# luizirber/sourmash-rust

Hardware: NVIDIA B200
Metric: Gbp/s sketched (higher is better)
Workload: dtype u64

## Files before the change

sourmash_rust_b200/csrc/kmer_bits.cuh:

```cuda
#pragma once
#include <stdint.h>

#if defined(__CUDACC__)
#define KB_HD __host__ __device__ __forceinline__
#else
#define KB_HD inline
#endif

namespace smb200 {

KB_HD uint32_t kb_byte_perm(uint32_t a, uint32_t b, uint32_t sel) {
#if defined(__CUDA_ARCH__)
    return __byte_perm(a, b, sel);
#else
    const uint64_t pool = ((uint64_t)b << 32) | a;
    uint32_t r = 0;
    for (int i = 0; i < 4; i++) {
        const uint32_t s = (sel >> (4 * i)) & 0x7u;
        r |= (uint32_t)((pool >> (8 * s)) & 0xFFu) << (8 * i);
    }
    return r;
#endif
}
KB_HD uint32_t kb_brev(uint32_t x) {
#if defined(__CUDA_ARCH__)
    return __brev(x);
#else
    x = ((x >> 1) & 0x55555555u) | ((x & 0x55555555u) << 1);
    x = ((x >> 2) & 0x33333333u) | ((x & 0x33333333u) << 2);
    x = ((x >> 4) & 0x0F0F0F0Fu) | ((x & 0x0F0F0F0Fu) << 4);
    x = ((x >> 8) & 0x00FF00FFu) | ((x & 0x00FF00FFu) << 8);
    return (x >> 16) | (x << 16);
#endif
}
KB_HD uint32_t kb_funnel_r(uint32_t lo, uint32_t hi, uint32_t s) {
#if defined(__CUDA_ARCH__)
    return __funnelshift_r(lo, hi, s);
#else
    s &= 31u;
    return s ? ((lo >> s) | (hi << (32 - s))) : lo;
#endif
}

struct Quad {
    uint32_t upper;
    uint32_t comp;
    uint32_t codes8;
    uint32_t bad4;
};
KB_HD Quad classify4(uint32_t raw) {
    Quad q;
    const uint32_t u = raw & 0xDFDFDFDFu;
    const uint32_t c = ((u >> 1) ^ (u >> 2)) & 0x03030303u;
    const uint32_t sel = (c & 0x3u) | ((c >> 4) & 0x30u) | ((c >> 8) & 0x300u) | ((c >> 12) & 0x3000u);
    const uint32_t expect = kb_byte_perm(0x54474341u , 0u, sel);
    const uint32_t x = expect ^ u;
    const uint32_t nz = (x | ((x & 0x7F7F7F7Fu) + 0x7F7F7F7Fu)) & 0x80808080u;
    q.upper = u;
    q.comp = kb_byte_perm(0x41434754u , 0u, sel);
    q.codes8 = (c * 0x01041040u) >> 24;
    q.bad4 = ((nz >> 7) * 0x01020408u) >> 24;
    return q;
}

KB_HD uint32_t pair_reverse16(uint32_t x) {
    x = kb_brev(x) >> 16;
    return ((x >> 1) & 0x5555u) | ((x & 0x5555u) << 1);
}

struct Oct {
    uint32_t fA0, fA1;
    uint32_t rA0, rA1;
    uint32_t f2;
    uint32_t r2;
    uint32_t bad8;
};
KB_HD Oct classify8(uint32_t raw0, uint32_t raw1) {
    const Quad a = classify4(raw0), b = classify4(raw1);
    Oct o;
    o.fA0 = a.upper;
    o.fA1 = b.upper;
    o.rA0 = kb_byte_perm(b.comp, 0u, 0x0123u);
    o.rA1 = kb_byte_perm(a.comp, 0u, 0x0123u);
    o.f2 = a.codes8 | (b.codes8 << 8);
    o.r2 = (~pair_reverse16(o.f2)) & 0xFFFFu;
    o.bad8 = a.bad4 | (b.bad4 << 4);
    return o;
}

template <int K>
struct KmerGeom {
    static constexpr int NE = (2 * K + 31) / 32;
    static constexpr int NW = (K + 3) / 4;
    static constexpr uint32_t TOP2 = (2 * K) % 32 ? ((1u << ((2 * K) % 32)) - 1u) : 0xFFFFFFFFu;
    static constexpr uint32_t TOPA = (K % 4) ? ((1u << ((K % 4) * 8)) - 1u) : 0xFFFFFFFFu;
};

template <int K>
KB_HD void extract2(const uint32_t *stream, int start, uint32_t (&e)[KmerGeom<K>::NE]) {
    const int w = start >> 4;
    const uint32_t s = (uint32_t)(start & 15) * 2u;
    uint32_t prev = stream[w];
#pragma unroll
    for (int j = 0; j < KmerGeom<K>::NE; j++) {
        const uint32_t next = stream[w + j + 1];
        e[j] = kb_funnel_r(prev, next, s);
        prev = next;
    }
    e[KmerGeom<K>::NE - 1] &= KmerGeom<K>::TOP2;
}

template <int K>
KB_HD void extract2w(const uint32_t *w, uint32_t s, uint32_t (&e)[KmerGeom<K>::NE]) {
    uint32_t prev = w[0];
#pragma unroll
    for (int j = 0; j < KmerGeom<K>::NE; j++) {
        const uint32_t next = w[j + 1];
        e[j] = kb_funnel_r(prev, next, s);
        prev = next;
    }
    e[KmerGeom<K>::NE - 1] &= KmerGeom<K>::TOP2;
}

template <int K>
KB_HD void extract2_end(const uint32_t *w, uint32_t s, uint32_t (&e)[KmerGeom<K>::NE]) {
    static_assert(K % 2 == 1, "end-aligned strand comparison needs an odd k");
    uint32_t prev = w[0];
#pragma unroll
    for (int j = 0; j < KmerGeom<K>::NE; j++) {
        const uint32_t next = w[j + 1];
        e[j] = kb_funnel_r(prev, next, s);
        prev = next;
    }
}

template <int K>
KB_HD bool canonical_is_fw(const uint32_t (&ef)[KmerGeom<K>::NE], const uint32_t (&er)[KmerGeom<K>::NE]) {
    constexpr int NE = KmerGeom<K>::NE;
    if (NE == 1) return ef[0] < er[0];
    if (NE == 2) return (((uint64_t)ef[1] << 32) | ef[0]) < (((uint64_t)er[1] << 32) | er[0]);
    bool lt = false;
#pragma unroll
    for (int j = 0; j < NE; j++) {
        if (ef[j] != er[j]) lt = ef[j] < er[j];
    }
    return lt;
}

template <int K>
KB_HD void extractA(const uint32_t *words, int start, uint32_t (&kw)[KmerGeom<K>::NW]) {
    const int w = start >> 2;
    const uint32_t s = (uint32_t)(start & 3) * 8u;
    uint32_t prev = words[w];
#pragma unroll
    for (int j = 0; j < KmerGeom<K>::NW; j++) {
        const uint32_t next = words[w + j + 1];
        kw[j] = kb_funnel_r(prev, next, s);
        prev = next;
    }
    kw[KmerGeom<K>::NW - 1] &= KmerGeom<K>::TOPA;
}

template <int K>
KB_HD void extractAw(const uint32_t *w, uint32_t s, uint32_t (&kw)[KmerGeom<K>::NW]) {
    uint32_t prev = w[0];
#pragma unroll
    for (int j = 0; j < KmerGeom<K>::NW; j++) {
        const uint32_t next = w[j + 1];
        kw[j] = kb_funnel_r(prev, next, s);
        prev = next;
    }
    kw[KmerGeom<K>::NW - 1] &= KmerGeom<K>::TOPA;
}

KB_HD void kb_shr96(uint32_t &x0, uint32_t &x1, uint32_t &x2, int s) {
    if (s < 32) {
        x0 = kb_funnel_r(x0, x1, (uint32_t)s);
        x1 = kb_funnel_r(x1, x2, (uint32_t)s);
        x2 >>= s;
    } else {
        x0 = kb_funnel_r(x1, x2, (uint32_t)(s - 32));
        x1 = (s == 32) ? x2 : (x2 >> (s - 32));
        x2 = 0;
    }
}
KB_HD uint32_t dilate_word(uint32_t in0, uint32_t in1, uint32_t in2, int span) {
    if (span <= 0) return 0;
    uint32_t d0 = in0, d1 = in1, d2 = in2;
    int a = 1;
    while (2 * a <= span) {
        uint32_t y0 = d0, y1 = d1, y2 = d2;
        kb_shr96(y0, y1, y2, a);
        d0 |= y0; d1 |= y1; d2 |= y2;
        a *= 2;
    }
    if (span > a) {
        uint32_t y0 = d0, y1 = d1, y2 = d2;
        kb_shr96(y0, y1, y2, span - a);
        d0 |= y0;
    }
    return d0;
}

}
```

sourmash_rust_b200/csrc/murmur3.cuh:

```cuda
#pragma once
#include <stdint.h>

#if defined(__CUDACC__)
#define SM_HD __host__ __device__ __forceinline__
#else
#define SM_HD inline
#endif

namespace smb200 {

constexpr uint64_t MM_C1 = 0x87c37b91114253d5ULL;
constexpr uint64_t MM_C2 = 0x4cf5ad432745937fULL;

template <uint64_t C>
SM_HD uint64_t mm_mulc(uint64_t x) {
#if defined(__CUDA_ARCH__)
    uint64_t r;
    asm("{\n\t.reg .u32 lo, hi, rl, rh;\n\t.reg .u64 t;\n\t"
        "mov.b64 {lo, hi}, %1;\n\t"
        "mul.wide.u32 t, lo, %2;\n\t"
        "mov.b64 {rl, rh}, t;\n\t"
        "mad.lo.u32 rh, lo, %3, rh;\n\t"
        "mad.lo.u32 rh, hi, %2, rh;\n\t"
        "mov.b64 %0, {rl, rh};\n\t}"
        : "=l"(r)
        : "l"(x), "n"((uint32_t)C), "n"((uint32_t)(C >> 32)));
    return r;
#else
    return x * C;
#endif
}
template <uint32_t ADD>
SM_HD uint64_t mm_mul5add(uint64_t x) {
#if defined(__CUDA_ARCH__) && defined(MM_MUL5_WIDE)
    uint64_t r;
    asm("{\n\t.reg .u32 lo, hi, rl, rh;\n\t.reg .u64 t;\n\t"
        "mov.b64 {lo, hi}, %1;\n\t"
        "mad.wide.u32 t, lo, 5, %2;\n\t"
        "mov.b64 {rl, rh}, t;\n\t"
        "mad.lo.u32 rh, hi, 5, rh;\n\t"
        "mov.b64 %0, {rl, rh};\n\t}"
        : "=l"(r)
        : "l"(x), "l"((uint64_t)ADD));
    return r;
#else
    return x * 5 + ADD;
#endif
}
template <int R>
SM_HD uint64_t mm_rotl64(uint64_t x) {
#if defined(__CUDA_ARCH__)
    const uint32_t lo = (uint32_t)x, hi = (uint32_t)(x >> 32);
    constexpr uint32_t S = (uint32_t)(R & 31);
    uint32_t nlo, nhi;
    if (R < 32) { nhi = __funnelshift_l(lo, hi, S); nlo = __funnelshift_l(hi, lo, S); }
    else        { nhi = __funnelshift_l(hi, lo, S); nlo = __funnelshift_l(lo, hi, S); }
    return ((uint64_t)nhi << 32) | nlo;
#else
    return (x << R) | (x >> (64 - R));
#endif
}

SM_HD uint64_t mm_xorshift33(uint64_t k) {
#if defined(__CUDA_ARCH__) && defined(MM_XS_IMADHI)
    uint32_t lo = (uint32_t)k, hi = (uint32_t)(k >> 32), t;
    asm("mul.hi.u32 %0, %1, 0x80000000;" : "=r"(t) : "r"(hi));
    lo ^= t;
    return ((uint64_t)hi << 32) | lo;
#else
    return k ^ (k >> 33);
#endif
}
SM_HD uint64_t mm_fmix64(uint64_t k) {
    k = mm_xorshift33(k);
    k = mm_mulc<0xff51afd7ed558ccdULL>(k);
    k = mm_xorshift33(k);
    k = mm_mulc<0xc4ceb9fe1a85ec53ULL>(k);
    k = mm_xorshift33(k);
    return k;
}

SM_HD uint64_t mm_mix_k1(uint64_t k1) {
    k1 = mm_mulc<MM_C1>(k1); k1 = mm_rotl64<31>(k1); k1 = mm_mulc<MM_C2>(k1);
    return k1;
}
SM_HD uint64_t mm_mix_k2(uint64_t k2) {
    k2 = mm_mulc<MM_C2>(k2); k2 = mm_rotl64<33>(k2); k2 = mm_mulc<MM_C1>(k2);
    return k2;
}
SM_HD void mm_body(uint64_t &h1, uint64_t &h2, uint64_t k1, uint64_t k2) {
    h1 ^= mm_mix_k1(k1);
    h1 = mm_rotl64<27>(h1); h1 += h2; h1 = mm_mul5add<0x52dce729u>(h1);
    h2 ^= mm_mix_k2(k2);
    h2 = mm_rotl64<31>(h2); h2 += h1; h2 = mm_mul5add<0x38495ab5u>(h2);
}
SM_HD uint64_t mm_final_h1(uint64_t h1, uint64_t h2, uint64_t len) {
    h1 ^= len; h2 ^= len;
    h1 += h2; h2 += h1;
    h1 = mm_fmix64(h1); h2 = mm_fmix64(h2);
    h1 += h2;
    return h1;
}

SM_HD uint64_t murmur3_h1_bytes(const uint8_t *data, uint64_t len, uint64_t seed) {
    uint64_t h1 = seed, h2 = seed;
    const uint64_t nblocks = len / 16;
    for (uint64_t b = 0; b < nblocks; b++) {
        uint64_t k1 = 0, k2 = 0;
        for (int j = 7; j >= 0; j--) {
            k1 = (k1 << 8) | data[16 * b + j];
            k2 = (k2 << 8) | data[16 * b + 8 + j];
        }
        mm_body(h1, h2, k1, k2);
    }
    const uint8_t *tail = data + nblocks * 16;
    const int rem = (int)(len & 15);
    uint64_t k1 = 0, k2 = 0;
    for (int j = rem - 1; j >= 8; j--) k2 = (k2 << 8) | tail[j];
    for (int j = (rem < 8 ? rem : 8) - 1; j >= 0; j--) k1 = (k1 << 8) | tail[j];
    if (rem > 8) h2 ^= mm_mix_k2(k2);
    if (rem > 0) h1 ^= mm_mix_k1(k1);
    return mm_final_h1(h1, h2, len);
}

template <int K>
SM_HD uint64_t murmur3_h1_words(const uint32_t *w, uint64_t seed) {
    constexpr int NB = K / 16;
    constexpr int REM = K % 16;
    uint64_t h1 = seed, h2 = seed;
#pragma unroll
    for (int b = 0; b < NB; b++) {
        const uint64_t k1 = ((uint64_t)w[4 * b + 1] << 32) | w[4 * b + 0];
        const uint64_t k2 = ((uint64_t)w[4 * b + 3] << 32) | w[4 * b + 2];
        mm_body(h1, h2, k1, k2);
    }
    if (REM > 8) {
        const uint32_t hi = (REM > 12) ? w[4 * NB + 3] : 0u;
        const uint64_t k2 = ((uint64_t)hi << 32) | w[4 * NB + 2];
        h2 ^= mm_mix_k2(k2);
    }
    if (REM > 0) {
        const uint32_t hi = (REM > 4) ? w[4 * NB + 1] : 0u;
        const uint64_t k1 = ((uint64_t)hi << 32) | w[4 * NB + 0];
        h1 ^= mm_mix_k1(k1);
    }
    return mm_final_h1(h1, h2, (uint64_t)K);
}

}
```

sourmash_rust_b200/csrc/sketch.cu:

```cuda
#include "device.hpp"
#include "kernels.cuh"
#include "kmer_bits.cuh"
#include "murmur3.cuh"

namespace smb200 {

#ifndef SK_UNROLL
#define SK_UNROLL 4
#endif
#ifndef SK_SHIFTED
#define SK_SHIFTED 1
#endif
#ifndef SK_UNROLL_FUSED
#define SK_UNROLL_FUSED 2
#endif
#ifndef SK_MIN_CTAS
#define SK_MIN_CTAS SK_CTAS_PER_SM
#endif

__device__ __forceinline__ uint32_t smem_u32(const void *p) { return (uint32_t)__cvta_generic_to_shared(p); }
__device__ __forceinline__ void mbar_init(uint64_t *bar, uint32_t count) {
    asm volatile("mbarrier.init.shared::cta.b64 [%0], %1;" ::"r"(smem_u32(bar)), "r"(count));
    asm volatile("fence.mbarrier_init.release.cluster;" ::: "memory");
}
__device__ __forceinline__ void mbar_expect_tx(uint64_t *bar, uint32_t bytes) {
    asm volatile("mbarrier.arrive.expect_tx.shared::cta.b64 _, [%0], %1;" ::"r"(smem_u32(bar)), "r"(bytes)
                 : "memory");
}
__device__ __forceinline__ void mbar_wait(uint64_t *bar, uint32_t parity) {
    asm volatile(
        "{\n\t"
        ".reg .pred p;\n\t"
        "WAIT_%=:\n\t"
        "mbarrier.try_wait.parity.shared::cta.b64 p, [%0], %1;\n\t"
        "@p bra DONE_%=;\n\t"
        "bra WAIT_%=;\n\t"
        "DONE_%=:\n\t"
        "}" ::"r"(smem_u32(bar)),
        "r"(parity)
        : "memory");
}
__device__ __forceinline__ void tma_load_1d(void *dst, const void *src, uint32_t bytes, uint64_t *bar) {
    asm volatile(
        "cp.async.bulk.shared::cluster.global.mbarrier::complete_tx::bytes [%0], [%1], %2, [%3];" ::"r"(
            smem_u32(dst)),
        "l"(src), "r"(bytes), "r"(smem_u32(bar))
        : "memory");
}

struct TileViews {
    uint8_t *raw;
    uint32_t *fA;
    uint32_t *rA;
    uint32_t *f2;
    uint32_t *r2;
    uint32_t *bad;
    uint32_t *end;
    uint32_t *sbad;
};
constexpr int SK_PAD2 = 4;
__host__ __device__ constexpr int tile_bases(int K) { return SK_TILE + ((K - 1 + 15) / 16) * 16; }
__host__ __device__ constexpr int copy_stride_words(int B) {
    int w = (B + 8) / 4 + 4;
    while (w % 32 != 8) w++;
    return w;
}
__host__ __device__ constexpr size_t tile_smem_bytes(int B, int nk = 1) {
    return (size_t)B
           + (SK_SHIFTED ? 8 * (size_t)copy_stride_words(B) * 4 : 2 * ((size_t)B + 16))
           + 2 * ((size_t)B / 4 + 8 + 4 * SK_PAD2)
           + 2 * ((size_t)(B + 31) / 32 * 4 + 12)
           + (size_t)nk * (SK_TILE / 8)
           + 128;
}
__device__ __forceinline__ TileViews carve_tile(uint8_t *base, int B) {
    TileViews v;
    uint8_t *p = base;
    v.raw = p; p += B;
    v.fA = reinterpret_cast<uint32_t *>(p); p += SK_SHIFTED ? 16 * copy_stride_words(B) : (B + 16);
    v.rA = reinterpret_cast<uint32_t *>(p); p += SK_SHIFTED ? 16 * copy_stride_words(B) : (B + 16);
    v.f2 = reinterpret_cast<uint32_t *>(p) + SK_PAD2; p += B / 4 + 8 + 4 * SK_PAD2;
    v.r2 = reinterpret_cast<uint32_t *>(p) + SK_PAD2; p += B / 4 + 8 + 4 * SK_PAD2;
    const int wm = (B + 31) / 32 + 3;
    v.bad = reinterpret_cast<uint32_t *>(p); p += wm * 4;
    v.end = reinterpret_cast<uint32_t *>(p); p += wm * 4;
    v.sbad = reinterpret_cast<uint32_t *>(p);
    return v;
}

__device__ __forceinline__ uint32_t tile_copy_bytes(uint64_t t0, uint64_t n, int B) {
    if (t0 >= n) return 0;
    const uint64_t left = ((n - t0) + 15) & ~15ull;
    return (uint32_t)(left < (uint64_t)B ? left : (uint64_t)B);
}

__device__ __forceinline__ void build_views(const TileViews &v, int B, uint64_t t0, const SketchBatch &sb) {
    const int tid = threadIdx.x, nthr = blockDim.x;
    const int wm = (B + 31) / 32 + 3;
    for (int w = tid; w < wm; w += nthr) v.end[w] = 0;
    for (int w = (B + 31) / 32 + tid; w < wm; w += nthr) v.bad[w] = 0xFFFFFFFFu;
    if (tid < 2) {
        v.fA[B / 4 + tid] = 0; v.rA[B / 4 + tid] = 0; v.f2[B / 16 + tid] = 0; v.r2[B / 16 + tid] = 0;
    }
    if (tid < SK_PAD2) { v.f2[-1 - tid] = 0; v.r2[-1 - tid] = 0; }
    const uint4 *raw128 = reinterpret_cast<const uint4 *>(v.raw);
    uint4 *fA128 = reinterpret_cast<uint4 *>(v.fA), *rA128 = reinterpret_cast<uint4 *>(v.rA);
    uint16_t *badh = reinterpret_cast<uint16_t *>(v.bad);
    const int groups = B / 16;
    for (int g = tid; g < groups; g += nthr) {
        const uint4 raw = raw128[g];
        const Oct o1 = classify8(raw.x, raw.y), o2 = classify8(raw.z, raw.w);
        uint32_t bad16 = o1.bad8 | (o2.bad8 << 8);
        const uint64_t b0 = t0 + (uint64_t)g * 16;
        if (b0 + 16 > sb.n) bad16 |= (b0 >= sb.n) ? 0xFFFFu : (0xFFFFu << (uint32_t)(sb.n - b0)) & 0xFFFFu;
        fA128[g] = make_uint4(o1.fA0, o1.fA1, o2.fA0, o2.fA1);
        const int rg = groups - 1 - g;
        rA128[rg] = make_uint4(o2.rA0, o2.rA1, o1.rA0, o1.rA1);
        v.f2[g] = o1.f2 | (o2.f2 << 16);
        v.r2[rg] = o2.r2 | (o1.r2 << 16);
        badh[g] = (uint16_t)bad16;
    }
    if (B % 32) {
        if (tid == 0) reinterpret_cast<uint16_t *>(v.bad)[B / 16] = 0xFFFFu;
    }
}

__device__ __forceinline__ void build_shifted_copies(const TileViews &v, int B) {
    const int quads = (B / 4 + 1 + 3) / 4, stride4 = copy_stride_words(B) / 4;
    for (int q = threadIdx.x; q < 2 * quads; q += blockDim.x) {
        uint32_t *x = (q < quads) ? v.fA : v.rA;
        const int j = (q < quads) ? q : q - quads;
        const uint4 a = reinterpret_cast<const uint4 *>(x)[j];
        const uint32_t n = x[4 * j + 4];
        uint4 *c = reinterpret_cast<uint4 *>(x);
#pragma unroll
        for (int s = 1; s < 4; s++)
            c[s * stride4 + j] = make_uint4(kb_funnel_r(a.x, a.y, 8 * s), kb_funnel_r(a.y, a.z, 8 * s), kb_funnel_r(a.z, a.w, 8 * s),
                                            kb_funnel_r(a.w, n, 8 * s));
    }
}

__device__ __forceinline__ void mark_sequence_ends(const TileViews &v, int B, uint64_t t0, const SketchBatch &sb) {
    const int tid = threadIdx.x, nthr = blockDim.x;
    const uint64_t hi = t0 + (uint64_t)B;
    if (sb.offsets == nullptr && sb.read_len == 0) {
        if (tid == 0 && sb.n - 1 >= t0 && sb.n - 1 < hi) {
            const uint32_t j = (uint32_t)(sb.n - 1 - t0);
            atomicOr(&v.end[j >> 5], 1u << (j & 31));
        }
    } else if (sb.offsets == nullptr) {
        if (tid < 32) {
            const uint64_t L = sb.read_len;
            uint64_t m = (t0 + 1 + L - 1) / L;
            if (m == 0) m = 1;
            for (m += tid;; m += 32) {
                const uint64_t e = m * L - 1;
                if (e >= hi || e >= sb.n) break;
                const uint32_t j = (uint32_t)(e - t0);
                atomicOr(&v.end[j >> 5], 1u << (j & 31));
            }
        }
    } else {
        uint64_t a = 0, b = sb.n_seqs;
        while (a < b) {
            const uint64_t mid = (a + b) >> 1;
            if (sb.offsets[mid + 1] > t0) b = mid; else a = mid + 1;
        }
        for (uint64_t s = a + tid; s < sb.n_seqs; s += nthr) {
            const uint64_t e1 = sb.offsets[s + 1];
            if (e1 - 1 >= hi) break;
            const uint32_t j = (uint32_t)(e1 - 1 - t0);
            atomicOr(&v.end[j >> 5], 1u << (j & 31));
        }
    }
}

__device__ __forceinline__ void build_start_bitmap(const TileViews &v, uint32_t *sbad, int K, uint64_t t0,
                                                   const SketchBatch &sb, unsigned long long *first_bad) {
    for (int w = threadIdx.x; w < SK_TILE / 32; w += blockDim.x) {
        uint32_t hasbad, crosses;
        if (K <= 64) {
            hasbad = dilate_word(v.bad[w], v.bad[w + 1], v.bad[w + 2], K);
            crosses = dilate_word(v.end[w], v.end[w + 1], v.end[w + 2], K - 1);
        } else {
            hasbad = 0; crosses = 0;
            for (int p = 0; p < 32; p++) {
                const int q = w * 32 + p;
                bool hb = false, cr = false;
                for (int j = q; j < q + K; j++) {
                    const uint32_t bit = 1u << (j & 31);
                    hb |= (v.bad[j >> 5] & bit) != 0;
                    if (j < q + K - 1) cr |= (v.end[j >> 5] & bit) != 0;
                }
                hasbad |= (uint32_t)hb << p;
                crosses |= (uint32_t)cr << p;
            }
        }
        const uint64_t q0 = t0 + (uint64_t)w * 32;
        uint32_t beyond = 0;
        if (q0 + 32 > sb.n_limit) beyond = (q0 >= sb.n_limit) ? 0xFFFFFFFFu : (0xFFFFFFFFu << (uint32_t)(sb.n_limit - q0));
        sbad[w] = hasbad | crosses | beyond;
        const uint32_t err = hasbad & ~crosses & ~beyond;
        if (err && first_bad)
            atomicMin(first_bad, (unsigned long long)(sb.pos_base + q0 + (uint32_t)(__ffs(err) - 1)));
    }
}

__device__ __forceinline__ void append_survivor(bool pass, uint64_t h, uint64_t pos0, const SketchBatch &sb,
                                                const SketchOut &out) {
    if (pass) {
        unsigned lane, tid;
        asm volatile("mov.u32 %0, %%laneid;" : "=r"(lane));
        asm volatile("mov.u32 %0, %%tid.x;" : "=r"(tid));
        const unsigned grp = __activemask();
        const int leader = __ffs(grp) - 1;
        unsigned long long base = 0;
        if ((int)lane == leader) base = atomicAdd(out.counter, (unsigned long long)__popc(grp));
        base = __shfl_sync(grp, base, leader);
        const unsigned long long idx = base + __popc(grp & ((1u << lane) - 1u));
        if (idx < out.cap) {
            out.hash[idx] = h;
            if (out.pos) out.pos[idx] = sb.pos_base + pos0 + tid;
        }
    }
}

template <int K, int B, int UNROLL>
__device__ __forceinline__ void kmer_loop(const TileViews &v, const uint32_t *sbad, const uint64_t thr, const uint64_t t0,
                                          const SketchBatch &sb, const SketchOut &out) {
    using G = KmerGeom<K>;
    static_assert(SK_THREADS % 32 == 0 && 16 * G::NE - K <= 16 * SK_PAD2, "k-mer loop addressing");
    const int tid = threadIdx.x;
    const int ri0 = B - K - tid, ra0 = B + 16 + ri0;
    const int ef0 = tid + K - 16 * G::NE, er0 = ri0 + K - 16 * G::NE;
    const uint32_t *qf2 = v.f2 + (ef0 >> 4), *qr2 = v.r2 + (er0 >> 4);
#if SK_SHIFTED
    constexpr int CS = copy_stride_words(B);
    const uint32_t *qfa = v.fA + (tid & 3) * CS + (tid >> 2), *qra = v.rA + (ri0 & 3) * CS + (ri0 >> 2);
    (void)ra0;
#else
    const uint32_t *qfa = v.fA + (tid >> 2), *qra = v.fA + (ra0 >> 2);
    const uint32_t sfa = (uint32_t)tid * 8u, sra = (uint32_t)ra0 * 8u;
#endif
    const uint32_t sf2 = (uint32_t)ef0 * 2u, sr2 = (uint32_t)er0 * 2u;
    const uint32_t *qsb = sbad + (tid >> 5);
    uint32_t mb = 1u << (tid & 31);
    asm("" : "+r"(mb));
#pragma unroll 1
    for (int r = 0; r < SK_TILE / SK_THREADS; r += UNROLL) {
#pragma unroll
        for (int u = 0; u < UNROLL; u++) {
            const bool valid = (qsb[u * (SK_THREADS / 32)] & mb) == 0;
            uint32_t ef[G::NE], er[G::NE];
            extract2_end<K>(qf2 + u * (SK_THREADS / 16), sf2, ef);
            extract2_end<K>(qr2 - u * (SK_THREADS / 16), sr2, er);
            const bool use_fw = canonical_is_fw<K>(ef, er);
            uint32_t kw[G::NW];
            const uint32_t *pa = use_fw ? qfa + u * (SK_THREADS / 4) : qra - u * (SK_THREADS / 4);
#if SK_SHIFTED
#pragma unroll
            for (int j = 0; j < G::NW; j++) kw[j] = pa[j];
            kw[G::NW - 1] &= G::TOPA;
#else
            extractAw<K>(pa, use_fw ? sfa : sra, kw);
#endif
            const uint64_t h = murmur3_h1_words<K>(kw, sb.seed);
            append_survivor(valid && h <= thr, h, t0 + (uint32_t)((r + u) * SK_THREADS), sb, out);
        }
        qf2 += UNROLL * (SK_THREADS / 16); qr2 -= UNROLL * (SK_THREADS / 16);
        qfa += UNROLL * (SK_THREADS / 4);  qra -= UNROLL * (SK_THREADS / 4);
        qsb += UNROLL * (SK_THREADS / 32);
    }
}

__host__ __device__ constexpr int kmax3(int a, int b, int c) { return a > b ? (a > c ? a : c) : (b > c ? b : c); }

template <int KA, int KB, int KC>
__global__ void __launch_bounds__(SK_THREADS, SK_MIN_CTAS) sketch_kernel(const SketchBatch sb, const SketchOuts outs,
                                                                         uint32_t n_tiles) {
    constexpr int B = tile_bases(kmax3(KA, KB, KC));
    extern __shared__ __align__(128) uint8_t s_dyn[];
    __shared__ __align__(8) uint64_t s_bar;
    const TileViews v = carve_tile(s_dyn, B);
    const int tid = threadIdx.x;
    const uint64_t thrA = *outs.o[0].thr;
    const uint64_t thrB = KB ? *outs.o[1].thr : 0;
    const uint64_t thrC = KC ? *outs.o[2].thr : 0;

    __shared__ uint32_t s_next;
    if (tid == 0) {
        mbar_init(&s_bar, 1);
        s_next = sb.tile_lo + gridDim.x + atomicAdd(sb.tile_ctr, 1u);
    }
    __syncthreads();
    uint32_t tile = sb.tile_lo + blockIdx.x;
    uint32_t parity = 0;
    if (tid == 0 && tile < n_tiles) {
        const uint64_t t0 = (uint64_t)tile * SK_TILE;
        const uint32_t bytes = tile_copy_bytes(t0, sb.n, B);
        mbar_expect_tx(&s_bar, bytes);
        if (bytes) tma_load_1d(v.raw, sb.buf + t0, bytes, &s_bar);
    }
    while (tile < n_tiles) {
        const uint64_t t0 = (uint64_t)tile * SK_TILE;
        const uint32_t next = s_next;
        uint32_t after_next = 0;
        mbar_wait(&s_bar, parity);
        parity ^= 1u;
        build_views(v, B, t0, sb);
        __syncthreads();
        if (tid == 0) {
            if (next < n_tiles) {
                const uint64_t n0 = (uint64_t)next * SK_TILE;
                const uint32_t bytes = tile_copy_bytes(n0, sb.n, B);
                mbar_expect_tx(&s_bar, bytes);
                if (bytes) tma_load_1d(v.raw, sb.buf + n0, bytes, &s_bar);
                after_next = sb.tile_lo + gridDim.x + atomicAdd(sb.tile_ctr, 1u);
            } else {
                after_next = next;
            }
        }
        mark_sequence_ends(v, B, t0, sb);
#if SK_SHIFTED
        build_shifted_copies(v, B);
#endif
        __syncthreads();
        build_start_bitmap(v, v.sbad, KA, t0, sb, outs.first_bad[0]);
        if (KB) build_start_bitmap(v, v.sbad + SK_TILE / 32, KB, t0, sb, outs.first_bad[1]);
        if (KC) build_start_bitmap(v, v.sbad + 2 * (SK_TILE / 32), KC, t0, sb, outs.first_bad[2]);
        __syncthreads();
        constexpr int U = KB ? SK_UNROLL_FUSED : SK_UNROLL;
        kmer_loop<KA, B, U>(v, v.sbad, thrA, t0, sb, outs.o[0]);
        if (KB) kmer_loop<(KB ? KB : KA), B, U>(v, v.sbad + SK_TILE / 32, thrB, t0, sb, outs.o[1]);
        if (KC) kmer_loop<(KC ? KC : KA), B, U>(v, v.sbad + 2 * (SK_TILE / 32), thrC, t0, sb, outs.o[2]);
        if (tid == 0) s_next = after_next;
        __syncthreads();
        tile = next;
    }
    if (tid == 0) {
        __threadfence();
        if (atomicAdd(sb.tile_ctr + 1, 1u) == gridDim.x - 1) {
            sb.tile_ctr[0] = 0;
            sb.tile_ctr[1] = 0;
            __threadfence();
        }
    }
}

__global__ void __launch_bounds__(SK_THREADS) sketch_generic_kernel(const SketchBatch sb, const SketchOut out,
                                                                    uint32_t n_tiles, int K) {
    const int B = SK_TILE + ((K - 1 + 15) / 16) * 16;
    extern __shared__ __align__(128) uint8_t s_dyn[];
    __shared__ __align__(8) uint64_t s_bar;
    const TileViews v = carve_tile(s_dyn, B);
    const int tid = threadIdx.x, lane = tid & 31;
    const uint64_t thr = *out.thr;
    if (tid == 0) mbar_init(&s_bar, 1);
    __syncthreads();
    uint32_t parity = 0;
    for (uint32_t tile = sb.tile_lo + blockIdx.x; tile < n_tiles; tile += gridDim.x) {
        const uint64_t t0 = (uint64_t)tile * SK_TILE;
        if (tid == 0) {
            const uint32_t bytes = tile_copy_bytes(t0, sb.n, B);
            mbar_expect_tx(&s_bar, bytes);
            if (bytes) tma_load_1d(v.raw, sb.buf + t0, bytes, &s_bar);
        }
        mbar_wait(&s_bar, parity);
        parity ^= 1u;
        build_views(v, B, t0, sb);
        __syncthreads();
        mark_sequence_ends(v, B, t0, sb);
        __syncthreads();
        build_start_bitmap(v, v.sbad, K, t0, sb, sb.first_bad);
        __syncthreads();
        const uint8_t *fA = reinterpret_cast<const uint8_t *>(v.fA);
        const uint8_t *rA = reinterpret_cast<const uint8_t *>(v.rA);
        for (int r = 0; r < SK_TILE / SK_THREADS; r++) {
            const int i = r * SK_THREADS + tid;
            const bool valid = ((v.sbad[i >> 5] >> (i & 31)) & 1u) == 0;
            uint64_t h = 0;
            if (valid) {
                const uint8_t *f = fA + i;
                const uint8_t *rc = rA + (B - K - i);
                int j = 0;
                while (j < K && f[j] == rc[j]) j++;
                const uint8_t *src = (j < K && f[j] < rc[j]) ? f : rc;
                h = murmur3_h1_bytes(src, (uint64_t)K, sb.seed);
            }
            append_survivor(valid && h <= thr, h, t0 + (uint32_t)(r * SK_THREADS), sb, out);
        }
        __syncthreads();
    }
}

bool sketch_has_fast_path(uint32_t K) { return K == 21 || K == 31 || K == 51; }
bool sketch_multi_supported(const uint32_t *ks, int nk) {
    if (nk < 2 || nk > 3) return false;
    for (int i = 0; i < nk; i++) {
        if (!sketch_has_fast_path(ks[i])) return false;
        if (i && ks[i] <= ks[i - 1]) return false;
    }
    return true;
}

template <int KA, int KB, int KC>
static void launch_fast(const SketchBatch &sb, const SketchOuts &outs, uint32_t n_tiles, unsigned grid, cudaStream_t st) {
    constexpr int NK = 1 + (KB ? 1 : 0) + (KC ? 1 : 0);
    constexpr size_t smem = tile_smem_bytes(tile_bases(kmax3(KA, KB, KC)), NK);
    static bool attr_set = false;
    if (!attr_set) {
        SM_CUDA(cudaFuncSetAttribute(sketch_kernel<KA, KB, KC>, cudaFuncAttributeMaxDynamicSharedMemorySize, (int)smem));
        attr_set = true;
    }
    sketch_kernel<KA, KB, KC><<<grid, SK_THREADS, smem, st>>>(sb, outs, n_tiles);
}

uint32_t sketch_tile_count(uint64_t n, uint64_t n_limit) {
    const uint64_t span = n_limit < n ? n_limit : n;
    const uint64_t tiles64 = (span + SK_TILE - 1) / SK_TILE;
    if (tiles64 > 0xFFFFFFFFull) throw_internal("sequence batch too large for one launch");
    return (uint32_t)tiles64;
}
uint32_t sketch_tiles_ready(uint32_t K, uint64_t bytes_ready) {
    const uint64_t B = SK_TILE + (((uint64_t)K - 1 + 15) / 16) * 16;
    if (bytes_ready < B) return 0;
    return (uint32_t)((bytes_ready - B) / SK_TILE + 1);
}

static unsigned sketch_grid(const SketchBatch &sb, uint32_t tile_hi, int sm_count) {
    unsigned grid = (unsigned)sm_count * SK_CTAS_PER_SM;
    if (grid > tile_hi - sb.tile_lo) grid = tile_hi - sb.tile_lo;
    return grid;
}

void launch_sketch(uint32_t K, const SketchBatch &sb, const SketchOut &out, uint32_t tile_hi, int sm_count,
                   cudaStream_t st) {
    if (sb.n == 0 || sb.n_limit == 0 || K == 0 || tile_hi <= sb.tile_lo) return;
    const uint32_t n_tiles = tile_hi;
    const unsigned grid = sketch_grid(sb, tile_hi, sm_count);
    ProfScope prof(K == 21 ? PROF_SKETCH_K21 : K == 31 ? PROF_SKETCH_K31 : K == 51 ? PROF_SKETCH_K51 : PROF_SKETCH_OTHER, st);
    SketchOuts outs;
    outs.o[0] = out; outs.o[1] = out; outs.o[2] = out;
    outs.first_bad[0] = sb.first_bad; outs.first_bad[1] = nullptr; outs.first_bad[2] = nullptr;
    switch (K) {
    case 21: launch_fast<21, 0, 0>(sb, outs, n_tiles, grid, st); break;
    case 31: launch_fast<31, 0, 0>(sb, outs, n_tiles, grid, st); break;
    case 51: launch_fast<51, 0, 0>(sb, outs, n_tiles, grid, st); break;
    default: {
        if (K > (uint32_t)SK_MAX_GENERIC_K) throw_internal("ksize above 8192 is not supported by the GPU sketcher");
        const int B = SK_TILE + (((int)K - 1 + 15) / 16) * 16;
        const size_t smem = tile_smem_bytes(B);
        SM_CUDA(cudaFuncSetAttribute(sketch_generic_kernel, cudaFuncAttributeMaxDynamicSharedMemorySize, (int)smem));
        sketch_generic_kernel<<<grid, SK_THREADS, smem, st>>>(sb, out, n_tiles, (int)K);
    }
    }
    SM_LAUNCHED();
}

void launch_sketch_multi(const uint32_t *ks, int nk, const SketchBatch &sb, const SketchOuts &outs, uint32_t tile_hi,
                         int sm_count, cudaStream_t st) {
    if (!sketch_multi_supported(ks, nk)) throw_internal("unsupported k-size combination for the fused sketch kernel");
    if (sb.n == 0 || sb.n_limit == 0 || tile_hi <= sb.tile_lo) return;
    const unsigned grid = sketch_grid(sb, tile_hi, sm_count);
    ProfScope prof(PROF_SKETCH_MULTI, st);
    if (nk == 3) launch_fast<21, 31, 51>(sb, outs, tile_hi, grid, st);
    else if (ks[0] == 21 && ks[1] == 31) launch_fast<21, 31, 0>(sb, outs, tile_hi, grid, st);
    else if (ks[0] == 21 && ks[1] == 51) launch_fast<21, 51, 0>(sb, outs, tile_hi, grid, st);
    else launch_fast<31, 51, 0>(sb, outs, tile_hi, grid, st);
    SM_LAUNCHED();
}

}
```

Before: 54.62.

## Share premixed murmur3 block words across k-sizes in fused 21/31/51 sketch kernel

For the fused k=21,31,51 kernel, each sub-tile now builds a shared-memory table of murmur3 k1/k2 mixes for every 8-byte-aligned forward and reverse-complement window. All three k-size loops then read these premixed words instead of recomputing the multiply-rotate mixes per k-mer, leaving only the tail bytes to mix inline. This drops the shifted-copy buffers for that path, adds per-sub-tile syncs and a larger smem footprint, and clamps the grid by the occupancy query.

```diff
diff --git a/sourmash_rust_b200/csrc/kmer_bits.cuh b/sourmash_rust_b200/csrc/kmer_bits.cuh
--- a/sourmash_rust_b200/csrc/kmer_bits.cuh
+++ b/sourmash_rust_b200/csrc/kmer_bits.cuh
@@ -173,6 +173,17 @@
     kw[KmerGeom<K>::NW - 1] &= KmerGeom<K>::TOPA;
 }
 
+template <int N>
+KB_HD uint64_t kb_bytes64(const uint32_t *w, uint32_t s) {
+    static_assert(N >= 1 && N <= 8, "1 to 8 bytes");
+    constexpr uint32_t LO = N >= 4 ? 0xFFFFFFFFu : (1u << (8 * N)) - 1u;
+    constexpr uint32_t HI = N <= 4 ? 0u : N == 8 ? 0xFFFFFFFFu : (1u << (8 * (N - 4))) - 1u;
+    const uint32_t x0 = w[0], x1 = w[1];
+    const uint32_t lo = kb_funnel_r(x0, x1, s) & LO;
+    const uint32_t hi = HI ? kb_funnel_r(x1, w[2], s) & HI : 0u;
+    return ((uint64_t)hi << 32) | lo;
+}
+
 KB_HD void kb_shr96(uint32_t &x0, uint32_t &x1, uint32_t &x2, int s) {
     if (s < 32) {
         x0 = kb_funnel_r(x0, x1, (uint32_t)s);
diff --git a/sourmash_rust_b200/csrc/murmur3.cuh b/sourmash_rust_b200/csrc/murmur3.cuh
--- a/sourmash_rust_b200/csrc/murmur3.cuh
+++ b/sourmash_rust_b200/csrc/murmur3.cuh
@@ -88,11 +88,14 @@
     k2 = mm_mulc<MM_C2>(k2); k2 = mm_rotl64<33>(k2); k2 = mm_mulc<MM_C1>(k2);
     return k2;
 }
+SM_HD void mm_body_mixed(uint64_t &h1, uint64_t &h2, uint64_t m1, uint64_t m2) {
+    h1 ^= m1;
+    h1 = mm_rotl64<27>(h1); h1 += h2; h1 = mm_mul5add<0x52dce729u>(h1);
+    h2 ^= m2;
+    h2 = mm_rotl64<31>(h2); h2 += h1; h2 = mm_mul5add<0x38495ab5u>(h2);
+}
 SM_HD void mm_body(uint64_t &h1, uint64_t &h2, uint64_t k1, uint64_t k2) {
-    h1 ^= mm_mix_k1(k1);
-    h1 = mm_rotl64<27>(h1); h1 += h2; h1 = mm_mul5add<0x52dce729u>(h1);
-    h2 ^= mm_mix_k2(k2);
-    h2 = mm_rotl64<31>(h2); h2 += h1; h2 = mm_mul5add<0x38495ab5u>(h2);
+    mm_body_mixed(h1, h2, mm_mix_k1(k1), mm_mix_k2(k2));
 }
 SM_HD uint64_t mm_final_h1(uint64_t h1, uint64_t h2, uint64_t len) {
     h1 ^= len; h2 ^= len;
@@ -147,4 +150,33 @@
     return mm_final_h1(h1, h2, (uint64_t)K);
 }
 
+struct MixPair {
+    uint64_t m1, m2;
+};
+SM_HD MixPair mm_mix_pair(uint64_t w0, uint64_t w1) {
+    MixPair e;
+    e.m1 = mm_mix_k1(w0);
+    e.m2 = mm_mix_k2(w1);
+    return e;
 }
+template <int K>
+struct PremixGeom {
+    static constexpr int NB = K / 16;
+    static constexpr int REM = K % 16;
+    static constexpr int NM = 2 * NB + (REM >= 8 ? 1 : 0);
+    static constexpr int TAIL_OFF = 8 * NM;
+    static constexpr int TAIL_LEN = K % 8;
+};
+template <int K>
+SM_HD uint64_t murmur3_h1_premixed(const uint64_t *m, uint64_t tail, uint64_t seed) {
+    using G = PremixGeom<K>;
+    uint64_t h1 = seed, h2 = seed;
+#pragma unroll
+    for (int b = 0; b < G::NB; b++) mm_body_mixed(h1, h2, m[2 * b], m[2 * b + 1]);
+    if (G::REM > 8) h2 ^= mm_mix_k2(tail);
+    if (G::REM >= 8) h1 ^= m[2 * G::NB];
+    else if (G::REM > 0) h1 ^= mm_mix_k1(tail);
+    return mm_final_h1(h1, h2, (uint64_t)K);
+}
+
+}
diff --git a/sourmash_rust_b200/csrc/sketch.cu b/sourmash_rust_b200/csrc/sketch.cu
--- a/sourmash_rust_b200/csrc/sketch.cu
+++ b/sourmash_rust_b200/csrc/sketch.cu
@@ -1,3 +1,5 @@
+#include <mutex>
+
 #include "device.hpp"
 #include "kernels.cuh"
 #include "kmer_bits.cuh"
@@ -16,6 +18,12 @@
 #endif
 #ifndef SK_MIN_CTAS
 #define SK_MIN_CTAS SK_CTAS_PER_SM
+#endif
+#ifndef SK_MIX_W
+#define SK_MIX_W 1024
+#endif
+#ifndef SK_MIX_UNROLL
+#define SK_MIX_UNROLL 4
 #endif
 
 __device__ __forceinline__ uint32_t smem_u32(const void *p) { return (uint32_t)__cvta_generic_to_shared(p); }
@@ -65,20 +73,20 @@
     while (w % 32 != 8) w++;
     return w;
 }
-__host__ __device__ constexpr size_t tile_smem_bytes(int B, int nk = 1) {
+__host__ __device__ constexpr size_t tile_smem_bytes(int B, int nk = 1, bool shifted = SK_SHIFTED) {
     return (size_t)B
-           + (SK_SHIFTED ? 8 * (size_t)copy_stride_words(B) * 4 : 2 * ((size_t)B + 16))
+           + (shifted ? 8 * (size_t)copy_stride_words(B) * 4 : 2 * ((size_t)B + 16))
            + 2 * ((size_t)B / 4 + 8 + 4 * SK_PAD2)
            + 2 * ((size_t)(B + 31) / 32 * 4 + 12)
            + (size_t)nk * (SK_TILE / 8)
            + 128;
 }
-__device__ __forceinline__ TileViews carve_tile(uint8_t *base, int B) {
+__device__ __forceinline__ TileViews carve_tile(uint8_t *base, int B, bool shifted = SK_SHIFTED) {
     TileViews v;
     uint8_t *p = base;
     v.raw = p; p += B;
-    v.fA = reinterpret_cast<uint32_t *>(p); p += SK_SHIFTED ? 16 * copy_stride_words(B) : (B + 16);
-    v.rA = reinterpret_cast<uint32_t *>(p); p += SK_SHIFTED ? 16 * copy_stride_words(B) : (B + 16);
+    v.fA = reinterpret_cast<uint32_t *>(p); p += shifted ? 16 * copy_stride_words(B) : (B + 16);
+    v.rA = reinterpret_cast<uint32_t *>(p); p += shifted ? 16 * copy_stride_words(B) : (B + 16);
     v.f2 = reinterpret_cast<uint32_t *>(p) + SK_PAD2; p += B / 4 + 8 + 4 * SK_PAD2;
     v.r2 = reinterpret_cast<uint32_t *>(p) + SK_PAD2; p += B / 4 + 8 + 4 * SK_PAD2;
     const int wm = (B + 31) / 32 + 3;
@@ -275,13 +283,96 @@
 
 __host__ __device__ constexpr int kmax3(int a, int b, int c) { return a > b ? (a > c ? a : c) : (b > c ? b : c); }
 
+__host__ __device__ constexpr bool sketch_uses_mix_table(int KA, int KB, int KC) { return KA == 21 && KB == 31 && KC == 51; }
+__host__ __device__ constexpr int mix_reach(int K) { return K <= 0 ? -(1 << 20) : (K % 16 >= 8 ? 16 * (K / 16) : 16 * (K / 16 - 1)); }
+__host__ __device__ constexpr int mix_rc_reach(int K) { return K <= 0 ? -(1 << 20) : mix_reach(K) - K; }
+template <int KA, int KB, int KC, int W>
+struct MixTile {
+    static constexpr int KMAX = kmax3(KA, KB, KC);
+    static constexpr int NF = W + kmax3(mix_reach(KA), mix_reach(KB), mix_reach(KC));
+    static constexpr int NR = W + KMAX + kmax3(mix_rc_reach(KA), mix_rc_reach(KB), mix_rc_reach(KC));
+    static constexpr int NT = NF + NR;
+    static constexpr size_t BYTES = ((size_t)NT * sizeof(MixPair) + 127) / 128 * 128;
+    __host__ __device__ static constexpr int rc_entry0(int K) { return NF + W - 1 + KMAX - K; }
+};
+
+template <int B, int NF, int NT>
+__device__ __forceinline__ void build_mix_table(const TileViews &v, MixPair *tab, int a, int rc_lo) {
+    for (int e = threadIdx.x; e < NT; e += blockDim.x) {
+        const int p = e < NF ? a + e : (B + 16) + rc_lo + (e - NF);
+        const uint32_t *w = v.fA + (p >> 2);
+        const uint32_t s = (uint32_t)p * 8u;
+        tab[e] = mm_mix_pair(kb_bytes64<8>(w, s), kb_bytes64<8>(w + 2, s));
+    }
+}
+
+template <int K, int B, int UNROLL, int W, int RC0>
+__device__ __forceinline__ void mix_loop(const TileViews &v, const MixPair *tab, const uint32_t *sbad, const uint64_t thr,
+                                         const uint64_t t0, const int a, const SketchBatch &sb, const SketchOut &out) {
+    using G = KmerGeom<K>;
+    using P = PremixGeom<K>;
+    static_assert(SK_THREADS % 32 == 0 && 16 * G::NE - K <= 16 * SK_PAD2, "k-mer loop addressing");
+    static_assert(W % (SK_THREADS * UNROLL) == 0 && SK_TILE % W == 0, "sub-tile shape");
+    const int tid = threadIdx.x;
+    const int i0 = a + tid, ri0 = B - K - i0, ra0 = B + 16 + ri0;
+    const int ef0 = i0 + K - 16 * G::NE, er0 = ri0 + K - 16 * G::NE;
+    const uint32_t *qf2 = v.f2 + (ef0 >> 4), *qr2 = v.r2 + (er0 >> 4);
+    const uint32_t sf2 = (uint32_t)ef0 * 2u, sr2 = (uint32_t)er0 * 2u;
+    const uint32_t *qfa = v.fA + (i0 >> 2) + P::TAIL_OFF / 4, *qra = v.fA + (ra0 >> 2) + P::TAIL_OFF / 4;
+    const uint32_t sfa = (uint32_t)i0 * 8u, sra = (uint32_t)ra0 * 8u;
+    const MixPair *tf = tab + tid, *tr = tab + RC0 - tid;
+    const uint32_t *qsb = sbad + (i0 >> 5);
+    uint32_t mb = 1u << (tid & 31);
+    asm("" : "+r"(mb));
+#pragma unroll 1
+    for (int r = 0; r < W / SK_THREADS; r += UNROLL) {
+#pragma unroll
+        for (int u = 0; u < UNROLL; u++) {
+            const bool valid = (qsb[u * (SK_THREADS / 32)] & mb) == 0;
+            uint32_t ef[G::NE], er[G::NE];
+            extract2_end<K>(qf2 + u * (SK_THREADS / 16), sf2, ef);
+            extract2_end<K>(qr2 - u * (SK_THREADS / 16), sr2, er);
+            const bool use_fw = canonical_is_fw<K>(ef, er);
+            const MixPair *pt = use_fw ? tf + u * SK_THREADS : tr - u * SK_THREADS;
+            uint64_t m[P::NM];
+#pragma unroll
+            for (int b = 0; b < P::NB; b++) {
+                const MixPair e = pt[16 * b];
+                m[2 * b] = e.m1;
+                m[2 * b + 1] = e.m2;
+            }
+            if (P::NM > 2 * P::NB) m[2 * P::NB] = pt[16 * P::NB].m1;
+            uint64_t tail = 0;
+            if (P::TAIL_LEN)
+                tail = kb_bytes64<(P::TAIL_LEN ? P::TAIL_LEN : 1)>(use_fw ? qfa + u * (SK_THREADS / 4) : qra - u * (SK_THREADS / 4),
+                                                                   use_fw ? sfa : sra);
+            const uint64_t h = murmur3_h1_premixed<K>(m, tail, sb.seed);
+            append_survivor(valid && h <= thr, h, t0 + (uint32_t)(a + (r + u) * SK_THREADS), sb, out);
+        }
+        qf2 += UNROLL * (SK_THREADS / 16); qr2 -= UNROLL * (SK_THREADS / 16);
+        qfa += UNROLL * (SK_THREADS / 4);  qra -= UNROLL * (SK_THREADS / 4);
+        tf += UNROLL * SK_THREADS;         tr -= UNROLL * SK_THREADS;
+        qsb += UNROLL * (SK_THREADS / 32);
+    }
+}
+
+template <int KA, int KB, int KC>
+__host__ __device__ constexpr size_t sketch_smem_bytes() {
+    return sketch_uses_mix_table(KA, KB, KC)
+               ? MixTile<KA, KB, KC, SK_MIX_W>::BYTES + tile_smem_bytes(tile_bases(kmax3(KA, KB, KC)), 1 + (KB ? 1 : 0) + (KC ? 1 : 0), false)
+               : tile_smem_bytes(tile_bases(kmax3(KA, KB, KC)), 1 + (KB ? 1 : 0) + (KC ? 1 : 0));
+}
+
 template <int KA, int KB, int KC>
 __global__ void __launch_bounds__(SK_THREADS, SK_MIN_CTAS) sketch_kernel(const SketchBatch sb, const SketchOuts outs,
                                                                          uint32_t n_tiles) {
     constexpr int B = tile_bases(kmax3(KA, KB, KC));
+    constexpr bool MIX = sketch_uses_mix_table(KA, KB, KC);
+    using MT = MixTile<KA, KB, KC, SK_MIX_W>;
     extern __shared__ __align__(128) uint8_t s_dyn[];
     __shared__ __align__(8) uint64_t s_bar;
-    const TileViews v = carve_tile(s_dyn, B);
+    MixPair *const tab = reinterpret_cast<MixPair *>(s_dyn);
+    const TileViews v = MIX ? carve_tile(s_dyn + MT::BYTES, B, false) : carve_tile(s_dyn, B);
     const int tid = threadIdx.x;
     const uint64_t thrA = *outs.o[0].thr;
     const uint64_t thrB = KB ? *outs.o[1].thr : 0;
@@ -321,20 +412,31 @@
             }
         }
         mark_sequence_ends(v, B, t0, sb);
-#if SK_SHIFTED
-        build_shifted_copies(v, B);
-#endif
+        if (SK_SHIFTED && !MIX) build_shifted_copies(v, B);
         __syncthreads();
         build_start_bitmap(v, v.sbad, KA, t0, sb, outs.first_bad[0]);
         if (KB) build_start_bitmap(v, v.sbad + SK_TILE / 32, KB, t0, sb, outs.first_bad[1]);
         if (KC) build_start_bitmap(v, v.sbad + 2 * (SK_TILE / 32), KC, t0, sb, outs.first_bad[2]);
-        __syncthreads();
-        constexpr int U = KB ? SK_UNROLL_FUSED : SK_UNROLL;
-        kmer_loop<KA, B, U>(v, v.sbad, thrA, t0, sb, outs.o[0]);
-        if (KB) kmer_loop<(KB ? KB : KA), B, U>(v, v.sbad + SK_TILE / 32, thrB, t0, sb, outs.o[1]);
-        if (KC) kmer_loop<(KC ? KC : KA), B, U>(v, v.sbad + 2 * (SK_TILE / 32), thrC, t0, sb, outs.o[2]);
-        if (tid == 0) s_next = after_next;
-        __syncthreads();
+        if constexpr (MIX) {
+            if (tid == 0) s_next = after_next;
+            constexpr int W = SK_MIX_W, KB_ = KB ? KB : KA, KC_ = KC ? KC : KA;
+            for (int a = 0; a < SK_TILE; a += W) {
+                build_mix_table<B, MT::NF, MT::NT>(v, tab, a, B - a - W + 1 - MT::KMAX);
+                __syncthreads();
+                mix_loop<KA, B, SK_MIX_UNROLL, W, MT::rc_entry0(KA)>(v, tab, v.sbad, thrA, t0, a, sb, outs.o[0]);
+                if (KB) mix_loop<KB_, B, SK_MIX_UNROLL, W, MT::rc_entry0(KB_)>(v, tab, v.sbad + SK_TILE / 32, thrB, t0, a, sb, outs.o[1]);
+                if (KC) mix_loop<KC_, B, SK_MIX_UNROLL, W, MT::rc_entry0(KC_)>(v, tab, v.sbad + 2 * (SK_TILE / 32), thrC, t0, a, sb, outs.o[2]);
+                __syncthreads();
+            }
+        } else {
+            __syncthreads();
+            constexpr int U = KB ? SK_UNROLL_FUSED : SK_UNROLL;
+            kmer_loop<KA, B, U>(v, v.sbad, thrA, t0, sb, outs.o[0]);
+            if (KB) kmer_loop<(KB ? KB : KA), B, U>(v, v.sbad + SK_TILE / 32, thrB, t0, sb, outs.o[1]);
+            if (KC) kmer_loop<(KC ? KC : KA), B, U>(v, v.sbad + 2 * (SK_TILE / 32), thrC, t0, sb, outs.o[2]);
+            if (tid == 0) s_next = after_next;
+            __syncthreads();
+        }
         tile = next;
     }
     if (tid == 0) {
@@ -403,16 +505,25 @@
     return true;
 }
 
+static unsigned sketch_grid(const SketchBatch &sb, uint32_t tile_hi, int sm_count, int ctas_per_sm = SK_CTAS_PER_SM) {
+    unsigned grid = (unsigned)sm_count * ctas_per_sm;
+    if (grid > tile_hi - sb.tile_lo) grid = tile_hi - sb.tile_lo;
+    return grid;
+}
+
 template <int KA, int KB, int KC>
-static void launch_fast(const SketchBatch &sb, const SketchOuts &outs, uint32_t n_tiles, unsigned grid, cudaStream_t st) {
-    constexpr int NK = 1 + (KB ? 1 : 0) + (KC ? 1 : 0);
-    constexpr size_t smem = tile_smem_bytes(tile_bases(kmax3(KA, KB, KC)), NK);
-    static bool attr_set = false;
-    if (!attr_set) {
+static void launch_fast(const SketchBatch &sb, const SketchOuts &outs, uint32_t tile_hi, int sm_count, cudaStream_t st) {
+    constexpr size_t smem = sketch_smem_bytes<KA, KB, KC>();
+    static std::once_flag attr_once;
+    static int ctas = SK_CTAS_PER_SM;
+    std::call_once(attr_once, [] {
         SM_CUDA(cudaFuncSetAttribute(sketch_kernel<KA, KB, KC>, cudaFuncAttributeMaxDynamicSharedMemorySize, (int)smem));
-        attr_set = true;
-    }
-    sketch_kernel<KA, KB, KC><<<grid, SK_THREADS, smem, st>>>(sb, outs, n_tiles);
+        int n = 0;
+        SM_CUDA(cudaOccupancyMaxActiveBlocksPerMultiprocessor(&n, sketch_kernel<KA, KB, KC>, SK_THREADS, smem));
+        if (n < 1) throw_internal("sketch kernel does not fit on an SM");
+        if (n < ctas) ctas = n;
+    });
+    sketch_kernel<KA, KB, KC><<<sketch_grid(sb, tile_hi, sm_count, ctas), SK_THREADS, smem, st>>>(sb, outs, tile_hi);
 }
 
 uint32_t sketch_tile_count(uint64_t n, uint64_t n_limit) {
@@ -427,31 +538,24 @@
     return (uint32_t)((bytes_ready - B) / SK_TILE + 1);
 }
 
-static unsigned sketch_grid(const SketchBatch &sb, uint32_t tile_hi, int sm_count) {
-    unsigned grid = (unsigned)sm_count * SK_CTAS_PER_SM;
-    if (grid > tile_hi - sb.tile_lo) grid = tile_hi - sb.tile_lo;
-    return grid;
-}
-
 void launch_sketch(uint32_t K, const SketchBatch &sb, const SketchOut &out, uint32_t tile_hi, int sm_count,
                    cudaStream_t st) {
     if (sb.n == 0 || sb.n_limit == 0 || K == 0 || tile_hi <= sb.tile_lo) return;
     const uint32_t n_tiles = tile_hi;
-    const unsigned grid = sketch_grid(sb, tile_hi, sm_count);
     ProfScope prof(K == 21 ? PROF_SKETCH_K21 : K == 31 ? PROF_SKETCH_K31 : K == 51 ? PROF_SKETCH_K51 : PROF_SKETCH_OTHER, st);
     SketchOuts outs;
     outs.o[0] = out; outs.o[1] = out; outs.o[2] = out;
     outs.first_bad[0] = sb.first_bad; outs.first_bad[1] = nullptr; outs.first_bad[2] = nullptr;
     switch (K) {
-    case 21: launch_fast<21, 0, 0>(sb, outs, n_tiles, grid, st); break;
-    case 31: launch_fast<31, 0, 0>(sb, outs, n_tiles, grid, st); break;
-    case 51: launch_fast<51, 0, 0>(sb, outs, n_tiles, grid, st); break;
+    case 21: launch_fast<21, 0, 0>(sb, outs, n_tiles, sm_count, st); break;
+    case 31: launch_fast<31, 0, 0>(sb, outs, n_tiles, sm_count, st); break;
+    case 51: launch_fast<51, 0, 0>(sb, outs, n_tiles, sm_count, st); break;
     default: {
         if (K > (uint32_t)SK_MAX_GENERIC_K) throw_internal("ksize above 8192 is not supported by the GPU sketcher");
         const int B = SK_TILE + (((int)K - 1 + 15) / 16) * 16;
         const size_t smem = tile_smem_bytes(B);
         SM_CUDA(cudaFuncSetAttribute(sketch_generic_kernel, cudaFuncAttributeMaxDynamicSharedMemorySize, (int)smem));
-        sketch_generic_kernel<<<grid, SK_THREADS, smem, st>>>(sb, out, n_tiles, (int)K);
+        sketch_generic_kernel<<<sketch_grid(sb, tile_hi, sm_count), SK_THREADS, smem, st>>>(sb, out, n_tiles, (int)K);
     }
     }
     SM_LAUNCHED();
@@ -461,12 +565,11 @@
                          int sm_count, cudaStream_t st) {
     if (!sketch_multi_supported(ks, nk)) throw_internal("unsupported k-size combination for the fused sketch kernel");
     if (sb.n == 0 || sb.n_limit == 0 || tile_hi <= sb.tile_lo) return;
-    const unsigned grid = sketch_grid(sb, tile_hi, sm_count);
     ProfScope prof(PROF_SKETCH_MULTI, st);
-    if (nk == 3) launch_fast<21, 31, 51>(sb, outs, tile_hi, grid, st);
-    else if (ks[0] == 21 && ks[1] == 31) launch_fast<21, 31, 0>(sb, outs, tile_hi, grid, st);
-    else if (ks[0] == 21 && ks[1] == 51) launch_fast<21, 51, 0>(sb, outs, tile_hi, grid, st);
-    else launch_fast<31, 51, 0>(sb, outs, tile_hi, grid, st);
+    if (nk == 3) launch_fast<21, 31, 51>(sb, outs, tile_hi, sm_count, st);
+    else if (ks[0] == 21 && ks[1] == 31) launch_fast<21, 31, 0>(sb, outs, tile_hi, sm_count, st);
+    else if (ks[0] == 21 && ks[1] == 51) launch_fast<21, 51, 0>(sb, outs, tile_hi, sm_count, st);
+    else launch_fast<31, 51, 0>(sb, outs, tile_hi, sm_count, st);
     SM_LAUNCHED();
 }
 
```

Measured after the change: 56.02, median of 6. 2.5% higher.
